# stschia/VAE-posterior-consistency

Hardware: AMD Instinct MI355X
Metric: training samples/sec (ELBO+consistency step), B=65536 d=128 (higher is better)
Workload: dtype f32; 1 GPU; Reg_VAE kl_reg alpha=1 beta=1 training step, synthetic tabular B=65536 per GPU, d=128, L=10, MCAR mask 0.7, p_missingness=30, Adam lr=1e-3, 8 resident batches rotated; global_batch=65536, parallelism=dp1

## Files before the change

### include/vpc.h

```cpp
#ifndef VPC_H
#define VPC_H
#include <stdint.h>

#ifdef __cplusplus
extern "C" {
#endif


int vpc_layout_sizes(int d, int L, int mask_augm, int* enc_img_floats, int* dec_img_floats, int* n_enc_params,
                     int* n_params, int* enc_part_floats, int* dec_part_floats, int* loss_terms, int* tile_rows);

int vpc_build_indices(int d, int L, int mask_augm, int* pack_idx, int* grad_idx, float* img_template);

int vpc_layout_sizes_pointnet(int d, int K, int L, int* enc_img_floats, int* dec_img_floats, int* n_enc_params, int* n_params,
                              int* n_front_params, int* enc_part_floats, int* dec_part_floats, int* loss_terms, int* tile_rows);
int vpc_build_indices_pointnet(int d, int K, int L, int* pack_idx, int* grad_idx, float* img_template);

int vpc_num_cus(void);
int vpc_max_partial_blocks(void);

int vpc_layout_sizes_bf16(int d, int L, int mask_augm, int* enc_img_floats, int* dec_img_floats);
int vpc_build_indices_bf16(int d, int L, int mask_augm, int* pack_idx_bf, float* img_template_bf);
int vpc_pack_weights_bf16(const float* flat_params, const int* pack_idx_bf, float* img_bf, int n, void* stream);

// ... 29 lines not shown
} VpcLossCoef;

int vpc_loss_fwd_bwd(const float* x, int npass, const float* const* xhat, const uint8_t* const* maskA,
                     const uint8_t* const* maskB, const VpcLossCoef* co, const float* const* mean,
                     const float* const* logvar, const float* eps_ml, float inv_B, float x_logvar,
                     float* const* dxhat, float* const* dmean, float* const* dlogvar, double* loss_partials,
                     int max_blocks, int* nblocks_out, long B, int d, int L, void* stream);

int vpc_decoder_fused(const float* x, const float* dec_img, int npass, const uint8_t* const* maskA,
                      const uint8_t* const* maskB, const VpcLossCoef* co, const float* const* mean,
                      const float* const* logvar, const float* const* eps, const float* eps_ml, float inv_B,
                      float x_logvar, float* const* dmean, float* const* dlogvar, int lat_pitch, int precision,
                      float* partials, double* loss_partials, int* nblocks_out, long B, int d, int L, void* stream);

int vpc_loss_finalize(const double* loss_partials, int nblocks, const VpcLossCoef* co, long B_local, long B_global,
                      int d, float* out9, float* accum, void* stream);

int vpc_build_inverse_maps(const int* grad_idx, int n_enc, int n, long enc_stride, long dec_stride, int* inv_out,
                           void* stream);
int vpc_reduce_step(const float* enc_partials, int enc_blocks, long enc_stride, const float* dec_partials,
                    int dec_blocks, long dec_stride, const int* grad_idx, const int* inv_maps, float* grad_out,
                    int n_enc, int n, const double* loss_partials, int loss_blocks, const VpcLossCoef* co, long B_local,
                    long B_global, int d, float* out9, float* accum, long long* state, long long rng_inc, void* stream);

int vpc_reduce_step_adam(const float* enc_partials, int enc_blocks, long enc_stride, const float* dec_partials,
                         int dec_blocks, long dec_stride, const int* grad_idx, const int* inv_maps, float* grad_out,
                         int n_enc, int n, const double* loss_partials, int loss_blocks, const VpcLossCoef* co,
                         long B_local, long B_global, int d, float* out9, float* accum, float* params, float* exp_avg,
                         float* exp_avg_sq, float lr, float beta1, float beta2, float eps, long step,
                         const int* pack_idx, float* img, void* stream);
int vpc_reduce_step_adam_bf16c(const float* enc_partials, int enc_blocks, long enc_stride, const float* dec_partials,
                         int dec_blocks, long dec_stride, const int* grad_idx, const int* inv_maps, float* grad_out,
                         int n_enc, int n, const double* loss_partials, int loss_blocks, const VpcLossCoef* co,
                         long B_local, long B_global, int d, float* out9, float* accum, float* params, float* exp_avg,
                         float* exp_avg_sq, float lr, float beta1, float beta2, float eps, long step,
                         const int* pack_idx_c, float* img_c, void* stream);


int vpc_draw_mask(const uint8_t* mask_in, uint8_t* mask_out, long n, float keep_prob, unsigned long long seed,
                  unsigned long long offset, long elem_lo, void* stream);

int vpc_draw_step(const uint8_t* mask_in, uint8_t* mask_out, long n_mask, float keep_prob, float* eps_out, long n_eps,
                  unsigned long long seed, unsigned long long offset_mask, unsigned long long offset_eps,
                  const long long* state, long mask_elem_lo, long eps_rows_local, long eps_rows_global,
                  long eps_row_lo, int eps_pitch, void* stream);

int vpc_fill_normal(float* out, long n, unsigned long long seed, unsigned long long offset, const long long* state,
                    long rows_local, long rows_global, long row_lo, int pitch, void* stream);

int vpc_encoder_fwd_draw_f32(const float* x, const float* enc_img, const uint8_t* mask_in, uint8_t* mask_p_out,
                             float* const* h1, float* const* h2, float* const* mean, float* const* logvar, long B, int d,
                             int L, float keep_prob, unsigned long long seed, unsigned long long offset_mask,
                             const long long* state, long mask_elem_lo, void* stream);
int vpc_decoder_fused_draw_f32(const float* x, const float* dec_img, int npass, const uint8_t* const* maskA,
                               const uint8_t* const* maskB, const VpcLossCoef* co, const float* const* mean,
                               const float* const* logvar, float* const* eps, float inv_B, float x_logvar,
                               float* const* dmean, float* const* dlogvar, float* partials, double* loss_partials,
                               int* nblocks_out, long B, int d, int L, unsigned long long seed,
                               unsigned long long offset_eps, const long long* state, long eps_rows_global, long eps_row_lo,
                               void* stream);

int vpc_rccl_unique_id(void* id128_host);
int vpc_rccl_comm_init(const void* id128_host, int nranks, int rank, void** comm_out);
int vpc_allreduce_flat(void* comm, float* bucket, long count, void* stream);
int vpc_rccl_comm_destroy(void* comm);

int vpc_reward_scratch(int n, int d, int M, long* pre_floats, long* stat_floats, long* w1t_floats);
int vpc_reward_matrix(const float* x, const uint8_t* mask, const float* im, const float* W1, const float* b1,
                      const float* enc_img, float* pre, float* stat, float* w1t, float* R, int n, int d, int L, int M,
                      void* stream);

#define VPC_REWARD_DENSE 0
#define VPC_REWARD_DENSE_MASK 1
#define VPC_REWARD_POINTNET 2
int vpc_reward_scratch_ex(int kind, int n, int d, int M, int K, long* pre_floats, long* stat_floats, long* w1t_floats);
int vpc_reward_matrix_ex(int kind, const float* x, const uint8_t* mask, const float* im, const float* W1, const float* b1,
                         const float* AC, int K, const float* w23_img, float* pre, float* stat, float* w1t, float* R, int n,
                         int d, int L, int M, void* stream);


int vpc_linear_fwd(const float* x, long ldx, const float* w, const float* bias, float* y, long ldy, long M, int N,
                   int K, int act, int act_split, int precision, void* stream);

int vpc_linear_dgrad(const float* dy, long lddy, const float* y_gate, long ldyg, int gate, int gate_split,
                     const float* w, const float* x_out, long ldx, int act_prev, float* dx, long lddx, long M, int N,
                     int K, int precision, void* stream);

long vpc_linear_wgrad_scratch(long M, int N, int K);
int vpc_linear_wgrad(const float* dy, long lddy, const float* y_gate, long ldyg, int gate, int gate_split,
                     const float* x, long ldx, float* dw, float* db, float* scratch, long scratch_floats, long M, int N,
                     int K, int accumulate, int precision, void* stream);
int vpc_linear_wgrad_reduce(int n_layers, const float* const* scratch, const long* M, const int* N, const int* K,
                            float* const* dw, float* const* db, const int* accumulate, void* stream);

int vpc_nm_sample(const float* heads, long ldh, const float* eps, float* z, long ldz, long B, int K, int L,
                  void* stream);
int vpc_nm_sample_bwd(const float* dz, long lddz, const float* eps, const float* heads, long ldh, const float* g_heads,
                      long ldg, float* out, long ldo, long B, int K, int L, void* stream);
int vpc_nm_mul(const float* x, const float* mask, float* out, long n, void* stream);

int vpc_nm_loss_blocks(long B);
long vpc_nm_loss_scratch(long B, int d);
int vpc_nm_loss(const float* x, const float* mask, const float* mask_p, const float* xm_q, const float* xl_q, long ld_q,
                const float* xm_p, const float* xl_p, long ld_p, const float* heads_q, const float* heads_p, long ldh,
                const float* W, const float* b, const float* eps_kl, float* g_xm_q, float* g_xl_q, long ldg_q,
                float* g_xm_p, float* g_xl_p, long ldg_p, float* g_heads_q, float* g_heads_p, long ldgh, float* gW,
// ... 270 lines not shown
```

### vae-posterior-consistency_amd/_lib.py

```python
from __future__ import annotations

import ctypes as C
import os
from functools import lru_cache

import numpy as np
import torch

_HERE = os.path.dirname(os.path.abspath(__file__))
LIB_PATH = os.environ.get("VPC_LIB") or os.path.join(_HERE, "csrc", "libvpc_hip.so")

_ERR = {1: "bad argument (null / misaligned pointer or bad count)", 2: "unsupported shape (beyond the limits of this entry point, include/vpc.h)",
        3: "HIP runtime error"}


class VpcError(RuntimeError):
    pass


P = C.c_void_p
PP = C.POINTER(C.c_void_p)
I = C.c_int
L_ = C.c_long
F = C.c_float
# ... 29 lines not shown
    "vpc_step_small_draw_f32": [P, P, P, I, PP, PP, P, PP, P, F, F, P, P, P, IP, L_, I, I, P, F, P, L_, ULL, ULL, ULL, P, L_, L_,
                                L_, L_, I, P],
    "vpc_step_small_aug_f32": [P, P, P, I, PP, PP, P, PP, P, F, F, P, P, P, IP, L_, I, I, I, P],
    "vpc_step_small_aug_draw_f32": [P, P, P, I, PP, PP, P, PP, P, F, F, P, P, P, IP, L_, I, I, I, P, F, P, L_, ULL, ULL, ULL, P, L_,
                                    L_, L_, L_, I, P],
    "vpc_step_small_eddi_f32": [P, P, P, I, PP, PP, P, PP, P, F, F, P, P, P, IP, L_, I, I, I, I, P, P, P, P],
    "vpc_step_small_eddi_draw_f32": [P, P, P, I, PP, PP, P, PP, P, F, F, P, P, P, IP, L_, I, I, I, I, P, P, P, P, F, P, L_, ULL, ULL,
                                     ULL, P, L_, L_, L_, L_, I, P],
    "vpc_reduce_step_adam_eddi": [P, I, L_, P, I, L_, P, P, I, P, I, P, L_, L_, I, P, P, P, P, P, F, F, F, F, L_, P, P, P, I, P, I,
                                  I, P],
    "vpc_step_small_multi_f32": [P, P, P, P, P, P, P, I, I, I, I, ULL, ULL, F, F, P, P, P, C.POINTER(L_), L_, I, I, I, P],
    "vpc_reduce_step_adam_multi": [P, P, P, I, L_, L_, C.POINTER(L_), P, P, I, P, L_, I, P, P, P, P, P, F, F, F, L_, P, P, P],
    "vpc_step_small_multi_aug_f32": [P, P, P, P, P, P, P, I, I, I, I, ULL, ULL, F, F, P, P, P, C.POINTER(L_), L_, I, I, I, I, P],
    "vpc_step_small_multi_eddi_f32": [P, P, P, P, P, P, P, I, I, I, I, ULL, ULL, F, F, P, P, P, C.POINTER(L_), L_, I, I, I, I, P, P,
                                      P, I, P],
    "vpc_reduce_step_adam_eddi_multi": [P, P, P, I, L_, L_, C.POINTER(L_), P, P, I, P, I, L_, I, P, P, P, P, P, F, F, F, L_, P, P, P,
                                        P, I, I, P],
    "vpc_eval_small_multi_f32": [P, P, P, P, P, P, I, P, L_, L_, L_, I, ULL, F, P, C.POINTER(L_), I, I, I, I, P],
    "vpc_eval_small_multi_aug_f32": [P, P, P, P, P, P, I, P, L_, L_, L_, I, ULL, F, P, C.POINTER(L_), I, I, I, I, P],
    "vpc_eval_small_multi_eddi_f32": [P, P, P, P, P, P, I, P, L_, L_, L_, I, ULL, F, P, C.POINTER(L_), I, I, I, I, P, I, P],
    "vpc_eval_reduce_multi": [P, P, L_, P, I, P, I, L_, L_, I, P, P],
    "vpc_impute_small_multi_f32": [P, P, P, P, P, P, I, P, L_, L_, L_, I, ULL, F, I, P, L_, C.POINTER(L_), I, I, I, I, P],
    "vpc_impute_small_multi_aug_f32": [P, P, P, P, P, P, I, P, L_, L_, L_, I, ULL, F, I, P, L_, C.POINTER(L_), I, I, I, I, P],
    "vpc_impute_small_multi_eddi_f32": [P, P, P, P, P, P, I, P, L_, L_, L_, I, ULL, F, I, P, L_, C.POINTER(L_), I, I, I, I, P, I,
                                        P],
    "vpc_target_mse_multi": [P, L_, L_, I, P, L_, P],
    "vpc_reward_scratch_multi_ex": [I, I, I, I, I, C.POINTER(L_), C.POINTER(L_), C.POINTER(L_)],
    "vpc_reward_matrix_multi_ex": [I, P, P, P, P, P, P, I, P, P, P, P, P, I, I, C.POINTER(L_), I, I, I, I, P],
    "vpc_eddi_fold_multi": [P, L_, P, L_, I, I, I, P],
    "vpc_reward_scratch_multi": [I, I, I, C.POINTER(L_), C.POINTER(L_), C.POINTER(L_)],
    "vpc_reward_matrix_multi": [P, P, P, P, P, P, P, P, P, P, I, I, C.POINTER(L_), I, I, I, I, P],
    "vpc_acquire_multi": [P, L_, P, L_, I, P, L_, I, P, L_, I, I, I, I, P],
    "vpc_step_fused_applicable": [L_, I, I, I],
    "vpc_step_layout_bf16": [I, I, IP, IP],
    "vpc_step_build_indices_bf16": [I, I, P, P],
    "vpc_step_pack_weights_bf16": [P, P, P, I, P],
    "vpc_step_workspace_floats": [L_],
    "vpc_step_fused_bf16": [P, P, I, PP, PP, P, PP, P, F, F, P, P, P, P, IP, L_, I, I, P],
    "vpc_encoder_fwd": [P, P, I, PP, PP, PP, PP, PP, PP, PP, I, I, I, L_, I, I, P],
    "vpc_encoder_bwd": [P, P, I, PP, PP, PP, PP, PP, I, I, I, P, IP, L_, I, I, P],
    "vpc_decoder_fwd": [P, P, P, L_, I, I, P],
    "vpc_decoder_bwd": [P, P, P, P, P, IP, L_, I, I, P],
    "vpc_loss_fwd_bwd": [P, I, PP, PP, PP, P, PP, PP, P, F, F, PP, PP, PP, P, I, IP, L_, I, I, P],
    "vpc_decoder_fused": [P, P, I, PP, PP, P, PP, PP, PP, P, F, F, PP, PP, I, I, P, P, IP, L_, I, I, P],
    "vpc_loss_finalize": [P, I, P, L_, L_, I, P, P, P],
    "vpc_build_inverse_maps": [P, I, I, L_, L_, P, P],
    "vpc_reduce_step": [P, I, L_, P, I, L_, P, P, P, I, I, P, I, P, L_, L_, I, P, P, P, C.c_longlong, P],
    "vpc_reduce_step_adam": [P, I, L_, P, I, L_, P, P, P, I, I, P, I, P, L_, L_, I, P, P, P, P, P, F, F, F, F, L_, P, P, P],
    "vpc_reduce_step_adam_bf16c": [P, I, L_, P, I, L_, P, P, P, I, I, P, I, P, L_, L_, I, P, P, P, P, P, F, F, F, F, L_, P, P, P],
    "vpc_draw_mask": [P, P, L_, F, ULL, ULL, L_, P],
    "vpc_draw_step": [P, P, L_, F, P, L_, ULL, ULL, ULL, P, L_, L_, L_, L_, I, P],
    "vpc_fill_normal": [P, L_, ULL, ULL, P, L_, L_, L_, I, P],
    "vpc_encoder_fwd_draw_f32": [P, P, P, P, PP, PP, PP, PP, L_, I, I, F, ULL, ULL, P, L_, P],
    "vpc_decoder_fused_draw_f32": [P, P, I, PP, PP, P, PP, PP, PP, F, F, PP, PP, P, P, IP, L_, I, I, ULL, ULL, P, L_, L_, P],
    "vpc_rccl_unique_id": [P],
    "vpc_rccl_comm_init": [P, I, I, PP],
    "vpc_allreduce_flat": [P, P, L_, P],
    "vpc_rccl_comm_destroy": [P],
    "vpc_reward_scratch": [I, I, I, C.POINTER(L_), C.POINTER(L_), C.POINTER(L_)],
    "vpc_reward_matrix": [P, P, P, P, P, P, P, P, P, P, I, I, I, I, P],
    "vpc_reward_scratch_ex": [I, I, I, I, I, C.POINTER(L_), C.POINTER(L_), C.POINTER(L_)],
    "vpc_reward_matrix_ex": [I, P, P, P, P, P, P, I, P, P, P, P, P, I, I, I, I, P],
    "vpc_linear_fwd": [P, L_, P, P, P, L_, L_, I, I, I, I, I, P],
    "vpc_linear_dgrad": [P, L_, P, L_, I, I, P, P, L_, I, P, L_, L_, I, I, I, P],
    "vpc_linear_wgrad_scratch": [L_, I, I],
    "vpc_linear_wgrad": [P, L_, P, L_, I, I, P, L_, P, P, P, L_, L_, I, I, I, I, P],
    "vpc_linear_wgrad_reduce": [I, PP, C.POINTER(L_), IP, IP, PP, PP, IP, P],
    "vpc_nm_sample": [P, L_, P, P, L_, L_, I, I, P],
    "vpc_nm_sample_bwd": [P, L_, P, P, L_, P, L_, P, L_, L_, I, I, P],
    "vpc_nm_mul": [P, P, P, L_, P],
    "vpc_nm_loss_blocks": [L_],
    "vpc_nm_loss_scratch": [L_, I],
    "vpc_nm_loss": [P, P, P, P, P, L_, P, P, L_, P, P, L_, P, P, P, P, P, L_, P, P, L_, P, P, L_, P, P, I, P, P, L_, P,
                    P, P, P, C.c_longlong, I, L_, L_, I, I, I, C.c_double, P],
    "vpc_nm_prep": [P, P, P, P, L_, I, F, P, L_, ULL, ULL, ULL, P, L_, L_, L_, L_, I, P],
    "vpc_nmdec_applicable": [L_, I, I, I],
    "vpc_nmdec_layout": [L_, I, I, I, IP, C.POINTER(C.c_long), IP],
    "vpc_nmdec_build_indices": [I, I, I, P, P, I],
    "vpc_nmenc_fwd": [P, P, P, P, P, L_, I, I, P],
    "vpc_nmenc_bwd": [P, P, P, P, P, P, L_, P, P, L_, I, I, P],
    "vpc_nmenc_build_indices": [I, I, I, P, C.POINTER(C.c_long), I],
    "vpc_nm_fused_bwd_step": [P, P, P, P, P, P, P, P, L_, P, P, P, P, P, L_, P, P, P, I, P, P, P, L_, L_, I, I, I, C.c_double,
                              P, P, P, F, F, F, F, L_, P, P],
    "vpc_nmdec_step": [P, P, P, P, P, L_, P, P, P, P, P, P, P, I, P, P, P, P, C.c_longlong, L_, L_, I, I, I, C.c_double, P],
    "vpc_miw_sample": [P, P, P, P, L_, I, I, P],
    "vpc_miw_sample_bwd": [P, P, P, P, P, L_, I, I, P],
    "vpc_miw_heads": [P, P, L_, I, P],
    "vpc_miw_heads_bwd": [P, P, P, L_, I, P],
    "vpc_miw_loss_scratch": [L_, I],
    "vpc_miw_loss": [P, P, P, P, P, L_, I, P, P, P, P, P, P, L_, P, P, P, P, L_, P, P, P, L_, I, I, I, C.c_double, I, P],
    "vpc_miw_small_workspace": [I, I],
    "vpc_miw_small_fwd": [P] * 11 + [L_, I, I, I, I, P],
    "vpc_miw_small_bwd": [P] * 13 + [L_, L_, I, I, I, I, P],
    "vpc_miw_small_tail": [P, L_, L_, I, I, I, P, P, P, P, F, F, F, F, L_, P],
    "vpc_miw_impute_scratch": [L_, I, I, I, I],
    "vpc_miw_impute": [P, P, P, P, ULL, ULL, L_, P, L_, P, P, L_, I, I, I, I, P],
    "vpc_miw_impute_draws": [P, L_, I, I, ULL, ULL, L_, P],
    "vpc_flow_prep": [P, P, P, P, P, P, L_, L_, I, F, ULL, ULL, ULL, P],
    "vpc_flow_fwd": [P, L_, P, P, P, L_, L_, P],
    "vpc_flow_bwd": [P, L_, P, P, P, P, P, L_, L_, L_, P],
    "vpc_flow_loss_scratch": [L_],
    "vpc_flow_loss": [P, P, P, P, P, L_, P, P, P, P, P, P, L_, P, P, P, P, P, L_, P, P, P, L_, I, I, F, F, F, I, P],
    "vpc_flow_reward_scratch": [I, I, I, I, I, C.POINTER(L_)],
    "vpc_flow_reward_matrix": [P, P, P, P, P, P, P, P, P, P, ULL, P, L_, P, I, I, I, I, I, P],
    "vpc_flow_reward_draws": [P, I, I, I, ULL, P],
    "vpc_ais_applicable": [L_, I, I],
# ... 173 lines not shown
```

### vae-posterior-consistency_amd/csrc/vpc_device.h

```cpp
#pragma once
#include <hip/hip_runtime.h>
#include <cstdint>
#include "vpc_layout.h"

namespace vpc {

typedef float f32x4 __attribute__((ext_vector_type(4)));

#define VPC_MFMA(a, b, c) __builtin_amdgcn_mfma_f32_16x16x4f32((a), (b), (c), 0, 0, 0)

__device__ __forceinline__ f32x4 zero4() { return f32x4{0.f, 0.f, 0.f, 0.f}; }
__device__ __forceinline__ float fast_sigmoid(float x) { return __builtin_amdgcn_rcpf(1.f + __expf(-x)); }
__device__ __forceinline__ f32x4 relu4(f32x4 v) {
    return f32x4{fmaxf(v[0], 0.f), fmaxf(v[1], 0.f), fmaxf(v[2], 0.f), fmaxf(v[3], 0.f)};
}
__device__ __forceinline__ f32x4 gate4(f32x4 dy, f32x4 act) {
    return f32x4{act[0] > 0.f ? dy[0] : 0.f, act[1] > 0.f ? dy[1] : 0.f, act[2] > 0.f ? dy[2] : 0.f,
                 act[3] > 0.f ? dy[3] : 0.f};
}

template <int T>
__device__ __forceinline__ uint32_t relu_bits(const f32x4 (&act)[T]) {
    uint32_t b = 0;
#pragma unroll
// ... 155 lines not shown
__device__ __forceinline__ void stage_bases(int (&sb)[4], int colbase, int c, int q) {
    const int col = colbase + c;
#pragma unroll
    for (int j = 0; j < 4; ++j) {
        const int f = 4 * q + j;
        sb[j] = f * CH + ((((col >> 2) ^ (f & stage_swz_mask<CH>())) << 2) | (col & 3));
    }
}
template <int CH>
__device__ __forceinline__ void stage_write_b(float* st, int t, f32x4 v, const int (&sb)[4]) {
#pragma unroll
    for (int j = 0; j < 4; ++j) st[16 * t * CH + sb[j]] = v[j];
}
template <int CH>
__device__ __forceinline__ f32x4 stage_frag(const float* st, int t, int s, int m, int q) {
    const int f = 16 * t + m;
    return *reinterpret_cast<const f32x4*>(st + f * CH + 4 * ((4 * s + q) ^ (f & stage_swz_mask<CH>())));
}

typedef const __attribute__((address_space(3))) f32x4* lds_f32x4_cptr;
typedef const __attribute__((address_space(3))) float* lds_f32_cptr;
__device__ __forceinline__ uint32_t lds_addr(const float* p) {
    return (uint32_t)(uintptr_t)(lds_f32_cptr)p;
}
__device__ __forceinline__ f32x4 lds_ld128(uint32_t addr) { return *(lds_f32x4_cptr)(uintptr_t)addr; }
__device__ __forceinline__ float lds_ld32(uint32_t addr) { return *(lds_f32_cptr)(uintptr_t)addr; }
template <int S>
__device__ __forceinline__ void frag_bases(uint32_t (&fb)[frag_nvar(S)], const float* W, int m, int q) {
    const uint32_t w0 = lds_addr(W);
#pragma unroll
    for (int v = 0; v < frag_nvar(S); ++v) {
        fb[v] = w0 + (uint32_t)frag_base(S, v, m, q);
        asm volatile("" : "+v"(fb[v]));
    }
}
template <int S, int OFF = 0>
__device__ __forceinline__ f32x4 frag_ld(const uint32_t (&fb)[frag_nvar(S)], int t, int s) {
    return lds_ld128(fb[frag_var(S, s)] + (uint32_t)(frag_imm(S, t, s) + OFF));
}
template <int KT, int S, int NK = 4 * KT>
__device__ __forceinline__ f32x4 tile_fwd_p2_b(const uint32_t (&fb)[frag_nvar(S)], int mt, const f32x4 (&in)[KT]) {
    f32x4 acc = zero4();
    f32x4 fa = frag_ld<S>(fb, mt, 0);
#pragma unroll
    for (int kt = 0; kt < KT; ++kt) {
        const f32x4 fn = kt + 1 < KT ? frag_ld<S>(fb, mt, kt + 1) : fa;
        __builtin_amdgcn_sched_barrier(0);
#pragma unroll
        for (int j = 0; j < 4; ++j)
            if (4 * kt + j < NK) acc = VPC_MFMA(fa[j], in[kt][j], acc);
        fa = fn;
    }
    return acc;
}
template <int S>
__device__ __forceinline__ void fragT_bases(uint32_t (&tj)[4], uint32_t (&tv)[fragT_nvar(S)], const float* W, int m, int q) {
    const uint32_t w0 = lds_addr(W);
#pragma unroll
    for (int j = 0; j < 4; ++j) {
        tj[j] = w0 + (uint32_t)fragT_base_j(S, j, m, q);
        asm volatile("" : "+v"(tj[j]));
    }
#pragma unroll
    for (int v = 0; v < fragT_nvar(S); ++v) {
        tv[v] = (uint32_t)fragT_base_v(S, v, q);
        asm volatile("" : "+v"(tv[v]));
    }
}
template <int KT, int S, int NK = 4 * KT>
__device__ __forceinline__ f32x4 tile_T_p2_b(const uint32_t (&tj)[4], const uint32_t (&tv)[fragT_nvar(S)], int mt,
                                             const f32x4 (&in)[KT]) {
    uint32_t p[4];
#pragma unroll
    for (int j = 0; j < 4; ++j) p[j] = tj[j] + tv[fragT_var(S, mt)];
    auto rd = [&](int kt) {
        f32x4 f;
#pragma unroll
        for (int j = 0; j < 4; ++j) f[j] = (4 * kt + j < NK) ? lds_ld32(p[j] + (uint32_t)fragT_imm(S, mt, kt)) : 0.f;
        return f;
    };
    f32x4 acc = zero4();
    f32x4 fa = rd(0);
#pragma unroll
    for (int kt = 0; kt < KT; ++kt) {
        const f32x4 fn = kt + 1 < KT ? rd(kt + 1) : fa;
        __builtin_amdgcn_sched_barrier(0);
#pragma unroll
        for (int j = 0; j < 4; ++j)
            if (4 * kt + j < NK) acc = VPC_MFMA(fa[j], in[kt][j], acc);
        fa = fn;
    }
    return acc;
}
template <int KT, int S, int NK = 4 * KT>
__device__ __forceinline__ f32x4 tile_T_b(const uint32_t (&tj)[4], const uint32_t (&tv)[fragT_nvar(S)], int mt,
                                          const f32x4 (&in)[KT], f32x4 acc) {
    uint32_t p[4];
#pragma unroll
    for (int j = 0; j < 4; ++j) p[j] = tj[j] + tv[fragT_var(S, mt)];
    float a[KT][4];
#pragma unroll
    for (int kt = 0; kt < KT; ++kt)
#pragma unroll
        for (int j = 0; j < 4; ++j)
            if (4 * kt + j < NK) a[kt][j] = lds_ld32(p[j] + (uint32_t)fragT_imm(S, mt, kt));
#pragma unroll
// ... 198 lines not shown
```

### vae-posterior-consistency_amd/csrc/vpc_enc.hip

```cpp
#include "vpc_device.h"
#include "vpc_bf16.h"
#include "vpc_abi_internal.h"
#include "vpc_rng.h"

namespace vpc {

template <bool VEC, bool AUG>
__device__ __forceinline__ f32x4 ld_input(const float* x, const uint8_t* mask, long row, int d, int t, int q, bool ok) {
    if (!AUG) {
        const f32x4 xv = ld_tile<VEC>(x, row, d, 16 * t + 4 * q, d, ok);
        const f32x4 mk = ld_mask<VEC>(mask, row, d, 16 * t + 4 * q, d, ok);
        return xv * mk;
    }
    f32x4 v;
#pragma unroll
    for (int j = 0; j < 4; ++j) {
        const int f = 16 * t + 4 * q + j;
        const bool isx = ok && f < d, ism = ok && f >= d && f < 2 * d;
        const long ix = isx ? row * d + f : 0, im = (isx || ism) ? row * d + (isx ? f : f - d) : 0;
        const float m = mask[im] ? 1.f : 0.f;
        v[j] = isx ? x[ix] * m : (ism ? m : 0.f);
    }
    return v;
}

struct EncFwdArgs {
    const float* x;
    const float* img;
    const uint8_t* mask[2];
    const float* eps[2];
    float* h1[2];
    float* h2[2];
    float* mean[2];
    float* logvar[2];
    float* z[2];
    long B;
    int d, L, npass, ntiles, lp;
    int psplit;
};
struct EncDraw {
    uint8_t* mask_out;
    float keep_prob;
    unsigned long long seed, off_mask;
    const long long* state;
    long elem_lo;
};

template <int DT, bool VEC, bool AUG, int NW, int PREC = PREC_F32>
__global__ __launch_bounds__(64 * NW, NW == 8 ? 2 : 1) void enc_fwd_kernel(EncFwdArgs a) {
    constexpr bool DRAW = false;
    const EncDraw dr{};
#include "vpc_enc_fwd_body.h"
}
template <int DT>
__global__ __launch_bounds__(512, 2) void enc_fwd_draw_kernel(EncFwdArgs a, EncDraw dr) {
    constexpr bool VEC = true, AUG = false, DRAW = true;
    constexpr int NW = 8, PREC = PREC_F32;
#include "vpc_enc_fwd_body.h"
}

struct EncBwdArgs {
    const float* x;
    const float* img;
    const uint8_t* mask[2];
    const float* h1[2];
    const float* h2[2];
    const float* dmean[2];
    const float* dlogvar[2];
    float* part;
    long B;
    int d, L, npass, ntiles, lp, dbg;
    int psplit;
};

#ifndef VPC_LANE_BASES
#define VPC_LANE_BASES 1
#endif

#ifdef VPC_ABLATE
#define ABLE(bit) ((a.dbg & (bit)) != 0)
#else
#define ABLE(bit) false
#endif

template <int DT, bool VEC, bool AUG, int NW, int PREC = PREC_F32>
__global__ __launch_bounds__(64 * NW, NW == 8 ? 2 : 1) void enc_bwd_kernel(EncBwdArgs a) {
    extern __shared__ __attribute__((aligned(16))) float lds[];
#ifdef VPC_ABLATE
    unsigned long long T[8] = {0, 0, 0, 0, 0, 0, 0, 0};
    unsigned long long tlast = __builtin_amdgcn_s_memtime();
#endif
    constexpr int TILE_ROWS = 16 * NW, CH = TILE_ROWS, NTHR = 64 * NW, OWN = 8 / NW;
    constexpr bool PIPE = VEC && !AUG;
    const EncImg im(DT);
    const int nW = im.total - im.oW2;
    float* W2 = lds;
    float* W3 = lds + (im.oW3 - im.oW2);
    float* stA = lds + nW;
    float* stB = stA + H1P * CH;
    float* db1s = stB + H1P * CH;
    constexpr bool BF = PREC != PREC_F32;
    constexpr int SKB = CH / 32;
    constexpr bool LB = !BF && NW == 8 && VPC_LANE_BASES;
    constexpr int OFF_B = H1P * CH * 4;
    static_assert(frag_imm(128, H1T - 1, 7) < 65536, "ds_read immediates are 16 bits");
    float* sAh = stA;
    float* sAl = stA + 56 * CH;
    float* sBh = stB;
    float* sBl = stB + 56 * CH;
    const int lane = threadIdx.x & 63, w = threadIdx.x >> 6, c = lane & 15, q = lane >> 4;
    const int ws = __builtin_amdgcn_readfirstlane(threadIdx.x >> 6);
// ... 315 lines not shown
                            __builtin_amdgcn_sched_barrier(0);
#pragma unroll
                            for (int j = 0; j < 4; ++j) acc1[o][mt] = VPC_MFMA(fa[j], fb[j], acc1[o][mt]);
                            fa = fn;
                        }
                    }
                }
            }
            VPC_STAMP(5);
        }
    }
#pragma unroll
    for (int mt = 0; mt < H1T; ++mt)
#pragma unroll
        for (int j = 0; j < 4; ++j) {
            float v = dbacc[mt][j];
            v += dpp_mov<0xB1>(v);
            v += dpp_mov<0x4E>(v);
            v += dpp_mov<0x141>(v);
            v += dpp_mov<0x140>(v);
            if (c == 0) db1s[w * 128 + 16 * mt + 4 * q + j] = v;
        }
    const long blk = (long)blockIdx.y * gridDim.x + blockIdx.x;
#pragma unroll
    for (int o = 0; o < OWN; ++o) {
        float* part = a.part + blk * ENC_PART + (long)(w + NW * o) * GREGS * 64 + lane;
#pragma unroll
        for (int mt = 0; mt < H1T; ++mt)
#pragma unroll
            for (int j = 0; j < 4; ++j) part[(4 * mt + j) * 64] = acc1[o][mt][j];
#pragma unroll
        for (int mt = 0; mt < H2T; ++mt)
#pragma unroll
            for (int j = 0; j < 4; ++j) part[(28 + 4 * mt + j) * 64] = acc2[o][mt][j];
#pragma unroll
        for (int j = 0; j < 4; ++j) part[(44 + j) * 64] = acc3[o][j];
    }
    __syncthreads();
    if (threadIdx.x < 128) {
        float t = 0.f;
#pragma unroll
        for (int k = 0; k < NW; ++k) t += db1s[k * 128 + threadIdx.x];
        a.part[blk * ENC_PART + WAVES * GREGS * 64 + threadIdx.x] = t;
    }
#ifdef VPC_ABLATE
    VPC_STAMP(6);
    if (ABLE(64) && blockIdx.x == 100 && (threadIdx.x & 63) == 0 && (threadIdx.x >> 6) % 3 == 0)
        printf("enc_bwd blk %d wave %d cycles: top %llu loads %llu dh2 %llu dW2 %llu dh1 %llu dW1+dW3 %llu epilogue %llu\n",
               blockIdx.x, (int)(threadIdx.x >> 6), T[0], T[1], T[2], T[3], T[4], T[5], T[6]);
#endif
}

static size_t enc_fwd_lds(int DT) { return sizeof(float) * EncImg(DT).total; }
static size_t enc_bwd_lds(int DT, int nw) {
    const EncImg im(DT);
    return sizeof(float) * ((im.total - im.oW2) + 2 * H1P * 16 * nw + nw * 128);
}

template <typename K, typename A>
static int launch(K kern, const A& args, int grid_x, int grid_y, int nw, size_t lds, hipStream_t stream) {
    if (!lds_attr_done(reinterpret_cast<const void*>(kern), lds)) return VPC_ERR_HIP;
    hipLaunchKernelGGL(kern, dim3(grid_x, grid_y), dim3(64 * nw), lds, stream, args);
    return hipGetLastError() == hipSuccess ? VPC_OK : VPC_ERR_HIP;
}

}

using namespace vpc;

extern "C" int vpc_encoder_fwd(const float* x, const float* enc_img, int npass, const uint8_t* const* mask,
                               const float* const* eps, float* const* h1, float* const* h2, float* const* mean,
                               float* const* logvar, float* const* z, int lat_pitch, int mask_augm, int precision,
                               long B, int d, int L, void* stream) {
    if (!x || !enc_img || !mask || !h1 || !h2 || !mean || !logvar) return VPC_ERR_ARG;
    if (npass < 1 || npass > 2 || B <= 0 || precision < 0 || precision > 2) return VPC_ERR_ARG;
    if (d < 1 || (mask_augm ? 2 * d : d) > MAX_D || L < 1 || L > MAX_L) return VPC_ERR_SHAPE;
    if (lat_pitch != L && lat_pitch != 16) return VPC_ERR_ARG;
    if (lat_pitch != L && z) return VPC_ERR_ARG;
    EncFwdArgs a{};
    a.x = x; a.img = enc_img; a.B = B; a.d = d; a.L = L; a.npass = npass; a.lp = lat_pitch;
    const TileShape ts = tile_shape(B, npass);
    a.ntiles = ts.ntiles; a.psplit = ts.small;
    bool vec = (d % 4 == 0) && aligned16(x);
    for (int p = 0; p < npass; ++p) {
        if (!mask[p] || !h1[p] || !h2[p] || !mean[p] || !logvar[p]) return VPC_ERR_ARG;
        a.mask[p] = mask[p]; a.eps[p] = eps ? eps[p] : nullptr; a.h1[p] = h1[p]; a.h2[p] = h2[p];
        a.mean[p] = mean[p]; a.logvar[p] = logvar[p]; a.z[p] = z ? z[p] : nullptr;
        vec = vec && ((uintptr_t)mask[p] % 4 == 0);
        if (!aligned16(h1[p]) || !aligned16(h2[p])) return VPC_ERR_ARG;
    }
    const int DT = dt_for(mask_augm ? 2 * d : d);
    const size_t lds = enc_fwd_lds(DT);
    hipStream_t s = (hipStream_t)stream;
    if (precision != PREC_F32) {
        if (!vec || mask_augm) return VPC_ERR_SHAPE;
#define VPC_CASE(T)                                                                                                    \
    case T:                                                                                                            \
        if (ts.small)                                                                                                  \
            return precision == PREC_BF16X3                                                                            \
                       ? launch(enc_fwd_kernel<T, true, false, 4, PREC_BF16X3>, a, ts.grid_x, ts.grid_y, 4, lds, s)    \
                       : launch(enc_fwd_kernel<T, true, false, 4, PREC_BF16>, a, ts.grid_x, ts.grid_y, 4, lds, s);     \
        return precision == PREC_BF16X3                                                                                \
                   ? launch(enc_fwd_kernel<T, true, false, 8, PREC_BF16X3>, a, ts.grid_x, ts.grid_y, 8, lds, s)        \
                   : launch(enc_fwd_kernel<T, true, false, 8, PREC_BF16>, a, ts.grid_x, ts.grid_y, 8, lds, s);
        switch (DT) { VPC_CASE(1) VPC_CASE(2) VPC_CASE(4) VPC_CASE(8) }
#undef VPC_CASE
        return VPC_ERR_SHAPE;
    }
#define VPC_LAUNCH(T, NW)                                                                                   \
    (mask_augm ? launch(enc_fwd_kernel<T, false, true, NW>, a, ts.grid_x, ts.grid_y, NW, lds, s)            \
     : vec     ? launch(enc_fwd_kernel<T, true, false, NW>, a, ts.grid_x, ts.grid_y, NW, lds, s)            \
               : launch(enc_fwd_kernel<T, false, false, NW>, a, ts.grid_x, ts.grid_y, NW, lds, s))
#define VPC_CASE(T) \
    case T: return ts.small ? VPC_LAUNCH(T, 4) : VPC_LAUNCH(T, 8);
    switch (DT) { VPC_CASE(1) VPC_CASE(2) VPC_CASE(4) VPC_CASE(8) }
#undef VPC_CASE
#undef VPC_LAUNCH
    return VPC_ERR_SHAPE;
}

extern "C" int vpc_encoder_fwd_draw_f32(const float* x, const float* enc_img, const uint8_t* mask_in, uint8_t* mask_p_out,
                                        float* const* h1, float* const* h2, float* const* mean, float* const* logvar, long B,
                                        int d, int L, float keep_prob, unsigned long long seed, unsigned long long offset_mask,
                                        const long long* state, long mask_elem_lo, void* stream) {
    if (!x || !enc_img || !mask_in || !mask_p_out || !h1 || !h2 || !mean || !logvar || B <= 0 || mask_elem_lo < 0) return VPC_ERR_ARG;
    if (d < 1 || d > MAX_D || L < 1 || L > MAX_L) return VPC_ERR_SHAPE;
    if (d % 8 != 0 || mask_elem_lo % 8 != 0 || dt_for(d) != 8 || !aligned16(x) || (uintptr_t)mask_in % 4 || (uintptr_t)mask_p_out % 4)
        return VPC_ERR_SHAPE;
    EncFwdArgs a{};
    a.x = x; a.img = enc_img; a.B = B; a.d = d; a.L = L; a.npass = 2; a.lp = 16;
    const TileShape ts = tile_shape(B, 2, true);
    a.ntiles = ts.ntiles; a.psplit = 0;
    for (int p = 0; p < 2; ++p) {
        if (!h1[p] || !h2[p] || !mean[p] || !logvar[p] || !aligned16(h1[p]) || !aligned16(h2[p])) return VPC_ERR_ARG;
        a.h1[p] = h1[p]; a.h2[p] = h2[p]; a.mean[p] = mean[p]; a.logvar[p] = logvar[p];
    }
    a.mask[0] = mask_in; a.mask[1] = mask_p_out;
    const EncDraw dr{mask_p_out, keep_prob, seed, offset_mask, state, mask_elem_lo};
    auto kern = enc_fwd_draw_kernel<8>;
    const size_t lds = enc_fwd_lds(8);
    if (!lds_attr_done(reinterpret_cast<const void*>(kern), lds)) return VPC_ERR_HIP;
    hipLaunchKernelGGL(kern, dim3(ts.grid_x), dim3(512), lds, (hipStream_t)stream, a, dr);
    return hipGetLastError() == hipSuccess ? VPC_OK : VPC_ERR_HIP;
}

extern "C" int vpc_encoder_bwd(const float* x, const float* enc_img, int npass, const uint8_t* const* mask,
                               const float* const* h1, const float* const* h2, const float* const* dmean,
                               const float* const* dlogvar, int lat_pitch, int mask_augm, int precision,
                               float* partials, int* nblocks_out, long B, int d, int L, void* stream) {
    if (!x || !enc_img || !mask || !h1 || !h2 || !dmean || !dlogvar || !partials) return VPC_ERR_ARG;
    if (npass < 1 || npass > 2 || B <= 0 || precision < 0 || precision > 2) return VPC_ERR_ARG;
    if (d < 1 || (mask_augm ? 2 * d : d) > MAX_D || L < 1 || L > MAX_L) return VPC_ERR_SHAPE;
    if (lat_pitch != L && lat_pitch != 16) return VPC_ERR_ARG;
    EncBwdArgs a{};
    a.x = x; a.img = enc_img; a.part = partials; a.B = B; a.d = d; a.L = L; a.npass = npass; a.lp = lat_pitch;
#ifdef VPC_ABLATE
    if (const char* e = getenv("VPC_DEBUG_ENC")) a.dbg = atoi(e);
#endif
    const TileShape ts = tile_shape(B, npass);
    a.ntiles = ts.ntiles; a.psplit = ts.small;
    bool vec = (d % 4 == 0) && aligned16(x);
    for (int p = 0; p < npass; ++p) {
        if (!mask[p] || !h1[p] || !h2[p] || !dmean[p] || !dlogvar[p]) return VPC_ERR_ARG;
        a.mask[p] = mask[p]; a.h1[p] = h1[p]; a.h2[p] = h2[p]; a.dmean[p] = dmean[p]; a.dlogvar[p] = dlogvar[p];
        vec = vec && ((uintptr_t)mask[p] % 4 == 0);
        if (!aligned16(h1[p]) || !aligned16(h2[p])) return VPC_ERR_ARG;
    }
    if (nblocks_out) *nblocks_out = ts.nblocks;
    const int DT = dt_for(mask_augm ? 2 * d : d);
    hipStream_t s = (hipStream_t)stream;
    if (precision != PREC_F32) {
        if (!vec || mask_augm) return VPC_ERR_SHAPE;
#define VPC_CASE(T)                                                                                                              \
    case T:                                                                                                                      \
        if (ts.small)                                                                                                            \
            return precision == PREC_BF16X3                                                                                      \
                       ? launch(enc_bwd_kernel<T, true, false, 4, PREC_BF16X3>, a, ts.grid_x, ts.grid_y, 4, enc_bwd_lds(T, 4), s) \
                       : launch(enc_bwd_kernel<T, true, false, 4, PREC_BF16>, a, ts.grid_x, ts.grid_y, 4, enc_bwd_lds(T, 4), s); \
        return precision == PREC_BF16X3                                                                                          \
                   ? launch(enc_bwd_kernel<T, true, false, 8, PREC_BF16X3>, a, ts.grid_x, ts.grid_y, 8, enc_bwd_lds(T, 8), s)    \
                   : launch(enc_bwd_kernel<T, true, false, 8, PREC_BF16>, a, ts.grid_x, ts.grid_y, 8, enc_bwd_lds(T, 8), s);
        switch (DT) { VPC_CASE(1) VPC_CASE(2) VPC_CASE(4) VPC_CASE(8) }
#undef VPC_CASE
        return VPC_ERR_SHAPE;
    }
#define VPC_LAUNCH(T, NW)                                                                                                  \
    (mask_augm ? launch(enc_bwd_kernel<T, false, true, NW>, a, ts.grid_x, ts.grid_y, NW, enc_bwd_lds(T, NW), s)            \
     : vec     ? launch(enc_bwd_kernel<T, true, false, NW>, a, ts.grid_x, ts.grid_y, NW, enc_bwd_lds(T, NW), s)            \
               : launch(enc_bwd_kernel<T, false, false, NW>, a, ts.grid_x, ts.grid_y, NW, enc_bwd_lds(T, NW), s))
#define VPC_CASE(T) \
    case T: return ts.small ? VPC_LAUNCH(T, 4) : VPC_LAUNCH(T, 8);
    switch (DT) { VPC_CASE(1) VPC_CASE(2) VPC_CASE(4) VPC_CASE(8) }
#undef VPC_CASE
#undef VPC_LAUNCH
    return VPC_ERR_SHAPE;
}
```

Measured before the change: 207.4 million samples/s.

## Add fused two-pass sweep encoder forward kernel sharing weight fragments across passes

Adds a new encoder-forward kernel that handles both passes (original mask and drawn consistency mask) in one sweep per tile. Each weight fragment loaded from LDS feeds two MFMA chains, one per pass, and the next tile's x and mask are prefetched into registers while the current tile computes. It is on by default for the draw path and opt-in through VPC_ENC_SWEEP for the non-draw path. Keeping two accumulator sets and the prefetched inputs raises register pressure, which could lower occupancy under launch_bounds(512,2).

```diff
diff --git a/include/vpc.h b/include/vpc.h
--- a/include/vpc.h
+++ b/include/vpc.h
@@ -105,6 +105,11 @@
                              float* const* h1, float* const* h2, float* const* mean, float* const* logvar, long B, int d,
                              int L, float keep_prob, unsigned long long seed, unsigned long long offset_mask,
                              const long long* state, long mask_elem_lo, void* stream);
+#define VPC_ENC_FWD_PASSES 0
+#define VPC_ENC_FWD_PASSES_DRAW 1
+#define VPC_ENC_FWD_SWEEP 2
+#define VPC_ENC_FWD_SWEEP_DRAW 3
+int vpc_encoder_fwd_last_form(void);
 int vpc_decoder_fused_draw_f32(const float* x, const float* dec_img, int npass, const uint8_t* const* maskA,
                                const uint8_t* const* maskB, const VpcLossCoef* co, const float* const* mean,
                                const float* const* logvar, float* const* eps, float inv_B, float x_logvar,
diff --git a/vae-posterior-consistency_amd/_lib.py b/vae-posterior-consistency_amd/_lib.py
--- a/vae-posterior-consistency_amd/_lib.py
+++ b/vae-posterior-consistency_amd/_lib.py
@@ -105,6 +105,7 @@
     "vpc_draw_step": [P, P, L_, F, P, L_, ULL, ULL, ULL, P, L_, L_, L_, L_, I, P],
     "vpc_fill_normal": [P, L_, ULL, ULL, P, L_, L_, L_, I, P],
     "vpc_encoder_fwd_draw_f32": [P, P, P, P, PP, PP, PP, PP, L_, I, I, F, ULL, ULL, P, L_, P],
+    "vpc_encoder_fwd_last_form": [],
     "vpc_decoder_fused_draw_f32": [P, P, I, PP, PP, P, PP, PP, PP, F, F, PP, PP, P, P, IP, L_, I, I, ULL, ULL, P, L_, L_, P],
     "vpc_rccl_unique_id": [P],
     "vpc_rccl_comm_init": [P, I, I, PP],
diff --git a/vae-posterior-consistency_amd/csrc/vpc_device.h b/vae-posterior-consistency_amd/csrc/vpc_device.h
--- a/vae-posterior-consistency_amd/csrc/vpc_device.h
+++ b/vae-posterior-consistency_amd/csrc/vpc_device.h
@@ -231,6 +231,35 @@
         fa = fn;
     }
     return acc;
+}
+template <int KT, int S, int MT, int NK, class Start, class Done>
+__device__ __forceinline__ void layer_fwd2_b(const uint32_t (&fb)[frag_nvar(S)], const f32x4 (&in0)[KT], const f32x4 (&in1)[KT],
+                                             Start start, Done done) {
+    static_assert(4 * (KT - 1) < NK && NK <= 4 * KT, "every k-tile holds at least one k-step");
+    f32x4 fa = frag_ld<S>(fb, 0, 0);
+    f32x4 st = start(0);
+#pragma unroll
+    for (int mt = 0; mt < MT; ++mt) {
+        f32x4 acc0 = st, acc1 = st;
+#pragma unroll
+        for (int kt = 0; kt < KT; ++kt) {
+            f32x4 fn = fa;
+            if (kt + 1 < KT) fn = frag_ld<S>(fb, mt, kt + 1);
+            else if (mt + 1 < MT) {
+                fn = frag_ld<S>(fb, mt + 1, 0);
+                st = start(mt + 1);
+            }
+            __builtin_amdgcn_sched_barrier(0);
+#pragma unroll
+            for (int j = 0; j < 4; ++j)
+                if (4 * kt + j < NK) {
+                    acc0 = VPC_MFMA(fa[j], in0[kt][j], acc0);
+                    acc1 = VPC_MFMA(fa[j], in1[kt][j], acc1);
+                }
+            fa = fn;
+        }
+        done(mt, acc0, acc1);
+    }
 }
 template <int S>
 __device__ __forceinline__ void fragT_bases(uint32_t (&tj)[4], uint32_t (&tv)[fragT_nvar(S)], const float* W, int m, int q) {
diff --git a/vae-posterior-consistency_amd/csrc/vpc_enc.hip b/vae-posterior-consistency_amd/csrc/vpc_enc.hip
--- a/vae-posterior-consistency_amd/csrc/vpc_enc.hip
+++ b/vae-posterior-consistency_amd/csrc/vpc_enc.hip
@@ -2,6 +2,8 @@
 #include "vpc_bf16.h"
 #include "vpc_abi_internal.h"
 #include "vpc_rng.h"
+#include <atomic>
+#include <cstdlib>
 
 namespace vpc {
 
@@ -57,6 +59,10 @@
     constexpr bool VEC = true, AUG = false, DRAW = true;
     constexpr int NW = 8, PREC = PREC_F32;
 #include "vpc_enc_fwd_body.h"
+}
+template <int DT, bool DRAW>
+__global__ __launch_bounds__(512, 2) void enc_fwd_sweep_kernel(EncFwdArgs a, EncDraw dr) {
+#include "vpc_enc_sweep_body.h"
 }
 
 struct EncBwdArgs {
@@ -478,6 +484,11 @@
 }
 
 static size_t enc_fwd_lds(int DT) { return sizeof(float) * EncImg(DT).total; }
+static bool enc_sweep_on(bool draw) {
+    const char* e = getenv("VPC_ENC_SWEEP");
+    return e ? atoi(e) != 0 : draw;
+}
+static std::atomic<int> enc_fwd_form{-1};
 static size_t enc_bwd_lds(int DT, int nw) {
     const EncImg im(DT);
     return sizeof(float) * ((im.total - im.oW2) + 2 * H1P * 16 * nw + nw * 128);
@@ -487,6 +498,13 @@
 static int launch(K kern, const A& args, int grid_x, int grid_y, int nw, size_t lds, hipStream_t stream) {
     if (!lds_attr_done(reinterpret_cast<const void*>(kern), lds)) return VPC_ERR_HIP;
     hipLaunchKernelGGL(kern, dim3(grid_x, grid_y), dim3(64 * nw), lds, stream, args);
+    return hipGetLastError() == hipSuccess ? VPC_OK : VPC_ERR_HIP;
+}
+
+template <typename K>
+static int launch(K kern, const EncFwdArgs& args, const EncDraw& dr, int grid_x, size_t lds, hipStream_t stream) {
+    if (!lds_attr_done(reinterpret_cast<const void*>(kern), lds)) return VPC_ERR_HIP;
+    hipLaunchKernelGGL(kern, dim3(grid_x), dim3(512), lds, stream, args, dr);
     return hipGetLastError() == hipSuccess ? VPC_OK : VPC_ERR_HIP;
 }
 
@@ -518,6 +536,9 @@
     const int DT = dt_for(mask_augm ? 2 * d : d);
     const size_t lds = enc_fwd_lds(DT);
     hipStream_t s = (hipStream_t)stream;
+    const bool sweep = precision == PREC_F32 && vec && !mask_augm && DT == 8 && npass == 2 && !ts.small && enc_sweep_on(false);
+    enc_fwd_form.store(sweep ? VPC_ENC_FWD_SWEEP : VPC_ENC_FWD_PASSES, std::memory_order_relaxed);
+    if (sweep) return launch(enc_fwd_sweep_kernel<8, false>, a, EncDraw{}, ts.grid_x, lds, s);
     if (precision != PREC_F32) {
         if (!vec || mask_augm) return VPC_ERR_SHAPE;
 #define VPC_CASE(T)                                                                                                    \
@@ -563,12 +584,17 @@
     }
     a.mask[0] = mask_in; a.mask[1] = mask_p_out;
     const EncDraw dr{mask_p_out, keep_prob, seed, offset_mask, state, mask_elem_lo};
+    const bool sweep = enc_sweep_on(true);
+    enc_fwd_form.store(sweep ? VPC_ENC_FWD_SWEEP_DRAW : VPC_ENC_FWD_PASSES_DRAW, std::memory_order_relaxed);
+    if (sweep) return launch(enc_fwd_sweep_kernel<8, true>, a, dr, ts.grid_x, enc_fwd_lds(8), (hipStream_t)stream);
     auto kern = enc_fwd_draw_kernel<8>;
     const size_t lds = enc_fwd_lds(8);
     if (!lds_attr_done(reinterpret_cast<const void*>(kern), lds)) return VPC_ERR_HIP;
     hipLaunchKernelGGL(kern, dim3(ts.grid_x), dim3(512), lds, (hipStream_t)stream, a, dr);
     return hipGetLastError() == hipSuccess ? VPC_OK : VPC_ERR_HIP;
 }
+
+extern "C" int vpc_encoder_fwd_last_form(void) { return enc_fwd_form.load(std::memory_order_relaxed); }
 
 extern "C" int vpc_encoder_bwd(const float* x, const float* enc_img, int npass, const uint8_t* const* mask,
                                const float* const* h1, const float* const* h2, const float* const* dmean,
diff --git a/vae-posterior-consistency_amd/csrc/vpc_enc_sweep_body.h b/vae-posterior-consistency_amd/csrc/vpc_enc_sweep_body.h
--- /dev/null
+++ b/vae-posterior-consistency_amd/csrc/vpc_enc_sweep_body.h
@@ -0,0 +1,169 @@
+    constexpr int NW = 8, TILE_ROWS = 16 * NW;
+    static_assert(DT == 8, "the sweep exists for d in (64, 128]");
+    extern __shared__ __attribute__((aligned(16))) float lds[];
+#ifdef VPC_ABLATE
+    unsigned long long T[8] = {0, 0, 0, 0, 0, 0, 0, 0};
+    unsigned long long tlast = __builtin_amdgcn_s_memtime();
+    const unsigned long long t_begin = tlast, r_begin = __builtin_amdgcn_s_memrealtime();
+#endif
+    constexpr int S1 = s_for_tiles(DT);
+    const EncImg im(DT);
+    const float* W1 = lds + im.oW1;
+    const float* b1 = lds + im.ob1;
+    const float* W2 = lds + im.oW2;
+    const float* W3 = lds + im.oW3;
+    const int lane = threadIdx.x & 63, w = threadIdx.x >> 6, c = lane & 15, q = lane >> 4;
+
+    f32x4 xraw[DT];
+    uint32_t mw[2][DT];
+    const int cq = (4 * q + 3 < a.d) ? 4 * q : 0;
+    const int vo = (w * 16 + c) * a.d + cq;
+    auto fetch_x = [&](long t0) {
+        const __amdgpu_buffer_rsrc_t rx = rows_rsrc(a.x, t0, a.B, a.d);
+#pragma unroll
+        for (int t = 0; t < DT; ++t)
+            xraw[t] = __builtin_bit_cast(f32x4, __builtin_amdgcn_raw_buffer_load_b128(
+                rx, 4 * (vo + ((t < DT / 2 || 16 * t + 4 * q + 3 < a.d) ? 16 * t : 0)), 0, 0));
+    };
+    auto fetch_m = [&](int p, long t0) {
+        const long rem = (a.B - t0) * (long)a.d;
+        const __amdgpu_buffer_rsrc_t rm = __builtin_amdgcn_make_buffer_rsrc(
+            const_cast<uint8_t*>(a.mask[p]) + t0 * a.d, 0, rem > 0xffffffffL ? 0xffffffffu : (uint32_t)rem, 0x00020000);
+#pragma unroll
+        for (int t = 0; t < DT; ++t)
+            mw[p][t] = (uint32_t)__builtin_amdgcn_raw_buffer_load_b32(
+                rm, vo + ((t < DT / 2 || 16 * t + 4 * q + 3 < a.d) ? 16 * t : 0), 0, 0);
+    };
+    auto fetch_tile = [&](long t0) {
+        fetch_x(t0);
+        fetch_m(0, t0);
+        if (!DRAW) fetch_m(1, t0);
+    };
+    uint64_t off_mask = 0;
+    if (DRAW) off_mask = dr.off_mask + (dr.state ? (uint64_t)dr.state[1] : 0);
+    if ((int)blockIdx.x < a.ntiles) fetch_tile((long)blockIdx.x * TILE_ROWS);
+    uint32_t keep[DRAW ? DT : 1];
+    auto draw_keep = [&](long r0, int qd) {
+        const int odd = qd & 1;
+        const uint32_t thr = mask_thr(dr.keep_prob);
+        const uint64_t g0 = off_mask + (uint64_t)mask_lane_group(dr.elem_lo, r0 + w * 16 + c, a.d, mask_lane_call_tile(0, qd), qd);
+#pragma unroll
+        for (int u = 0; u < DT / 2; ++u) {
+            const U4 r = philox(g0 + 4 * u, 0u, dr.seed);
+            const uint32_t o0 = odd ? r.z : r.x, o1 = odd ? r.w : r.y, s0 = odd ? r.x : r.z, s1 = odd ? r.y : r.w;
+            const uint32_t r0w = (uint32_t)__builtin_amdgcn_ds_swizzle((int)s0, 0x401F);
+            const uint32_t r1w = (uint32_t)__builtin_amdgcn_ds_swizzle((int)s1, 0x401F);
+            const uint32_t kown = keep_bits4(o0, o1, thr), koth = keep_bits4(r0w, r1w, thr);
+            keep[2 * u] = odd ? koth : kown;
+            keep[2 * u + 1] = odd ? kown : koth;
+        }
+#pragma unroll
+        for (int t = 0; t < (DRAW ? DT : 1); ++t) asm volatile("" : "+v"(keep[t]));
+    };
+    load_image<13>(lds, a.img, im.total);
+    __syncthreads();
+    VPC_STAMP(0);
+
+    for (int tile = blockIdx.x; tile < a.ntiles; tile += gridDim.x) {
+        const long row = (long)tile * TILE_ROWS + w * 16 + c;
+        const bool ok = row < a.B;
+        asm volatile("" ::: "memory");
+        int cc = c, qq = q;
+        launder(cc, qq);
+        const long row0 = (long)tile * TILE_ROWS;
+        const int lrow = w * 16 + c;
+        f32x4 xin[2][DT];
+        if (DRAW) {
+            draw_keep(row0, qq);
+            const long mrem = (a.B - row0) * (long)a.d;
+            const __amdgpu_buffer_rsrc_t ro = __builtin_amdgcn_make_buffer_rsrc(
+                dr.mask_out + row0 * a.d, 0, mrem > 0xffffffffL ? 0xffffffffu : (uint32_t)mrem, 0x00020000);
+#pragma unroll
+            for (int t = 0; t < DT; ++t) {
+                mw[1][t] = mw[0][t] & keep[DRAW ? t : 0];
+                asm volatile("" : "+v"(mw[1][t]));
+                if (t < DT / 2 || 16 * t + 4 * q + 3 < a.d)
+                    __builtin_amdgcn_raw_buffer_store_b32((int)mw[1][t], ro, vo + 16 * t, 0, 0);
+            }
+            __builtin_amdgcn_sched_barrier(0);
+        }
+#pragma unroll
+        for (int t = 0; t < DT; ++t) {
+            const uint32_t vm = opaque_mask(t < DT / 2 || 16 * t + 4 * q + 3 < a.d);
+            xin[0][t] = xraw[t] * mask_to_f32(mw[0][t] & vm);
+            xin[1][t] = xraw[t] * mask_to_f32(mw[1][t] & vm);
+        }
+        if (tile + (int)gridDim.x < a.ntiles) fetch_tile(row0 + (long)gridDim.x * TILE_ROWS);
+        VPC_STAMP(1);
+        f32x4 h1[2][H1T], h2[2][H2T], ml[2][2];
+        {
+            const __amdgpu_buffer_rsrc_t r0 = rows_rsrc(a.h1[0], row0, a.B, H1P), r1 = rows_rsrc(a.h1[1], row0, a.B, H1P);
+            uint32_t f1[4];
+            frag_bases<S1>(f1, W1, cc, qq);
+            uint32_t bb = lds_addr(b1) + 16u * (uint32_t)qq;
+            asm volatile("" : "+v"(bb));
+            layer_fwd2_b<DT, S1, H1T, 4 * DT>(
+                f1, xin[0], xin[1], [&](int mt) { return lds_ld128(bb + 64u * mt); },
+                [&](int mt, f32x4 acc0, f32x4 acc1) {
+                    h1[0][mt] = relu4(acc0);
+                    h1[1][mt] = relu4(acc1);
+                    st_rows(r0, lrow, H1P, 16 * mt + 4 * q, h1[0][mt]);
+                    st_rows(r1, lrow, H1P, 16 * mt + 4 * q, h1[1][mt]);
+                });
+        }
+        VPC_STAMP(2);
+        launder(cc, qq);
+        {
+            const __amdgpu_buffer_rsrc_t r0 = rows_rsrc(a.h2[0], row0, a.B, H2P), r1 = rows_rsrc(a.h2[1], row0, a.B, H2P);
+            uint32_t f2[4];
+            frag_bases<128>(f2, W2, cc, qq);
+            layer_fwd2_b<H1T, 128, H2T, NK1>(
+                f2, h1[0], h1[1], [&](int) { return zero4(); },
+                [&](int mt, f32x4 acc0, f32x4 acc1) {
+                    h2[0][mt] = relu4(acc0);
+                    h2[1][mt] = relu4(acc1);
+                    st_rows(r0, lrow, H2P, 16 * mt + 4 * q, h2[0][mt]);
+                    st_rows(r1, lrow, H2P, 16 * mt + 4 * q, h2[1][mt]);
+                });
+        }
+        VPC_STAMP(3);
+        launder(cc, qq);
+        {
+            uint32_t f3[4];
+            frag_bases<64>(f3, W3, cc, qq);
+            layer_fwd2_b<H2T, 64, 2, NK2>(
+                f3, h2[0], h2[1], [&](int) { return zero4(); },
+                [&](int mt, f32x4 acc0, f32x4 acc1) {
+                    ml[0][mt] = acc0;
+                    ml[1][mt] = acc1;
+                });
+        }
+#pragma unroll
+        for (int p = 0; p < 2; ++p) {
+            const f32x4 mu = ml[p][0], lv = ml[p][1];
+            if (a.lp == 16) {
+                st_rows(rows_rsrc(a.mean[p], row0, a.B, 16), lrow, 16, 4 * q, mu);
+                st_rows(rows_rsrc(a.logvar[p], row0, a.B, 16), lrow, 16, 4 * q, lv);
+            } else {
+                st_tile<false>(a.mean[p], row, a.L, 4 * q, a.L, ok, mu);
+                st_tile<false>(a.logvar[p], row, a.L, 4 * q, a.L, ok, lv);
+            }
+            if (a.z[p]) {
+                f32x4 z = mu;
+                if (a.eps[p]) {
+                    const f32x4 e = ld_tile<false>(a.eps[p], row, a.L, 4 * q, a.L, ok);
+#pragma unroll
+                    for (int j = 0; j < 4; ++j) z[j] = mu[j] + e[j] * expf(lv[j] * 0.5f);
+                }
+                st_tile<false>(a.z[p], row, a.L, 4 * q, a.L, ok, z);
+            }
+        }
+        VPC_STAMP(4);
+    }
+#ifdef VPC_ABLATE
+    if ((blockIdx.x == 0 || blockIdx.x == 100) && (threadIdx.x & 63) == 0 && (threadIdx.x >> 6) < 2)
+        printf("enc_fwd sweep blk %d wave %d cycles: prologue %llu loadx %llu L1 %llu L2 %llu L3+st %llu | total %llu cycles in %llu x 10 ns\n",
+               blockIdx.x, (int)(threadIdx.x >> 6), T[0], T[1], T[2], T[3], T[4],
+               (unsigned long long)(__builtin_amdgcn_s_memtime() - t_begin),
+               (unsigned long long)(__builtin_amdgcn_s_memrealtime() - r_begin));
+#endif
```

Result: faster. 211.1 million samples/s, median of 6 (+1.8%).
